# thierrydumas/autoencoder_based_image_compression

Measured on AMD Instinct MI355X. Metric: Mpixels/s encode+decode (Kodak 768x512 luma), bitstream bit-exact, higher is better.
Workload: dtype f32; 1 GPU; kodak_512x768_luma_batch24_per_gpu_bin_width_1.0_lossless_roundtrip; height=512, width=768, truncated_unary_length=10, idx_map_exception=67, parallelism=single GPU, coder=device, 64 maps per wavefront, encode + decode + compare

## Files before the change

autoencoder_based_image_compression_amd/csrc/hip/coder_simd.hip:

```cpp
#include <hip/hip_runtime.h>
#include <stdint.h>

#include <mutex>

#include "../coder/lean_step.h"
#include "eae_hip.h"
#include "fill.h"
#include "wave_scan.h"

int eae_coder_generic_encode(uint32_t n_maps, uint32_t map_size, const int16_t* symbols, uint8_t L, const double* probs,
                             const int32_t* prob_row, uint8_t* streams, uint64_t stride, uint32_t* bac_bits,
                             uint32_t* bypass_bits, int32_t* status, int32_t* stage, int only_status, hipStream_t stream);
int eae_coder_generic_decode(uint32_t n_maps, uint32_t map_size, int16_t* out, uint8_t L, const double* probs,
                             const int32_t* prob_row, const uint8_t* streams, uint64_t stride, const uint32_t* bac_bits,
                             const uint32_t* bypass_bits, int32_t* status, int32_t* stage, int only_status, hipStream_t stream);

#ifndef EAE_RES_BINARISE
#define EAE_RES_BINARISE 47
#endif
#ifndef EAE_RES_ENCODE_CORE
#define EAE_RES_ENCODE_CORE 55
#endif
#ifndef EAE_RES_EMIT
#define EAE_RES_EMIT 39
#endif
#ifndef EAE_RES_DECODE_CORE
#define EAE_RES_DECODE_CORE 55
#endif
#ifndef EAE_RES_DEBINARISE
#define EAE_RES_DEBINARISE 23
#endif
#ifndef EAE_RES_DEBINARISE_STAGED
#define EAE_RES_DEBINARISE_STAGED 39
#endif
#ifndef EAE_RES_DECODE_CORE_CHUNKED
#define EAE_RES_DECODE_CORE_CHUNKED 63
#endif
#ifndef EAE_DECODE_TOPUP_ZEROS
#define EAE_KEEP_VGPR_FREE_(n) asm volatile("; v" #n " reserved: the last register of the allocation holds no operand" ::: "v" #n)
#define EAE_KEEP_LAST_VGPR_FREE(n) EAE_KEEP_VGPR_FREE_(n)
#else
#define EAE_KEEP_LAST_VGPR_FREE(n)
#endif

namespace {

using namespace eae_core;
using namespace eae_lean;


#ifndef EAE_SIMD_PRIO
#define EAE_SIMD_PRIO 3
#endif

constexpr int32_t RETRY = -100;
constexpr uint32_t kMaxFastL = 32;
constexpr uint32_t kRecordPad = 12;
constexpr uint32_t kRing = 32;
constexpr uint32_t kBypassStage = 512;
constexpr uint32_t kDebinariseStage = 1024;
constexpr uint32_t kEmitWords = 224;

struct SimdParams {
    uint32_t n_maps, map_size, L, dcap;
    uint32_t rcap;
    const int16_t* symbols;
    int16_t* decoded;
    const double* probs;
    const int32_t* prob_row;
    uint8_t* streams;
    uint64_t stride;
    uint32_t* bac_bits;
    uint32_t* bypass_bits;
    int32_t* status;
    int32_t* stage;
    uint8_t* decisions;
    uint32_t* ndec;
    uint32_t* records;
    uint8_t* prefixes;
    uint32_t chunk, nchunks;
    uint32_t* group_steps;
    uint2* enc_state;
    uint4* emit_state;
    uint32_t* avail_bits;
    uint4* dec_state;
    uint2* dec_state2;
};

__host__ __device__ inline uint32_t chunk_span(uint32_t steps, uint32_t nchunks) {
    const uint32_t span = ((steps + nchunks - 1u) / nchunks + 63u) & ~63u;
    return span ? span : 64u;
}

__device__ __forceinline__ int wave_exclusive_max(int v) {
    int m = __builtin_amdgcn_update_dpp(-1, v, 0x138, 0xF, 0xF, false);
#define EAE_MAX_STEP(ctrl_, rows_)                                                        \
    {                                                                                     \
        const int o_ = __builtin_amdgcn_update_dpp(-1, m, ctrl_, rows_, 0xF, false);      \
        m = o_ > m ? o_ : m;                                                              \
    }
    EAE_MAX_STEP(0x111, 0xF)
    EAE_MAX_STEP(0x112, 0xF)
    EAE_MAX_STEP(0x114, 0xF)
    EAE_MAX_STEP(0x118, 0xF)
    EAE_MAX_STEP(0x142, 0xA)
    EAE_MAX_STEP(0x143, 0xC)
#undef EAE_MAX_STEP
    return m;
}
__device__ __forceinline__ uint32_t wave_max(uint32_t v) {
#pragma unroll
    for (int d = 32; d >= 1; d >>= 1) {
        const uint32_t o = __shfl_xor(v, d, 64);
        v = o > v ? o : v;
    }
    return v;
}

__global__ __launch_bounds__(64) void binarise_kernel(const SimdParams p) {
    EAE_KEEP_LAST_VGPR_FREE(EAE_RES_BINARISE);
    __shared__ unsigned long long ybuf[40];
    const uint32_t m = blockIdx.x, lane = threadIdx.x;
    const int32_t row = p.prob_row ? p.prob_row[m] : (int32_t)m;
    if (row < 0) {
        if (lane == 0) { p.ndec[m] = 0; p.bac_bits[m] = 0; p.bypass_bits[m] = 0; p.status[m] = 0; if (p.stage) p.stage[m] = 0; }
        return;
    }
    const uint32_t L = p.L;
    const int16_t* in = p.symbols + (size_t)m * p.map_size;
    uint8_t* dec = p.decisions + (size_t)(m >> 6) * 64u * p.dcap + (size_t)(m & 63u) * 8u;
    unsigned long long* ystream = reinterpret_cast<unsigned long long*>(p.streams + (uint64_t)m * p.stride + p.stride / 2);
    const uint32_t size_bits = round_up_to_byte(required_bits(p.map_size, L));
    uint32_t jbase = 0, bbase = 0;
    bool overflow = false;
    if (lane < 40) ybuf[lane] = 0;
    for (uint32_t t = 0; t < p.map_size; t += 64) {
        const uint32_t i = t + lane;
        const bool valid = i < p.map_size;
        const int s = valid ? (int)in[i] : 0;
        const uint32_t a = (uint32_t)(s < 0 ? -s : s);
        const uint32_t ones = a < L ? a : L;
        const uint32_t nd = valid ? ones + (a < L ? 1u : 0u) : 0u;
        unsigned long long bb = 0;
        uint32_t nb = 0;
        if (valid && a >= L) {
            const uint32_t v = a - L + 1u;
            const uint32_t n = count_nb_bits(v) - 1u;
            bb = ((1ull << n) - 1ull) | ((unsigned long long)(n ? rev16(v - (1u << n)) >> (16u - n) : 0u) << (n + 1u));
            nb = 2u * n + 1u;
        }
        if (valid && s != 0) {
            bb |= (unsigned long long)(s > 0 ? 1u : 0u) << nb;
            nb++;
        }
        uint32_t both_tot;
        const uint32_t both = wave_exclusive_scan(nd | (nb << 16), both_tot);
        const uint32_t jo = both & 0xFFFFu, bo = both >> 16, jtot = both_tot & 0xFFFFu, btot = both_tot >> 16;
        for (uint32_t q = 0; q < nd; q++) {
            const uint32_t j = jbase + jo + q;
            dec[(size_t)(j >> 3) * 512u + (j & 7u)] = (uint8_t)((q << 1) | (q < ones ? 1u : 0u));
        }
        if (nb) {
            const uint32_t pos = (bbase & 63u) + bo;
            atomicOr(&ybuf[pos >> 6], bb << (pos & 63u));
            if ((pos & 63u) + nb > 64u) atomicOr(&ybuf[(pos >> 6) + 1u], bb >> (64u - (pos & 63u)));
        }
        if (bbase + btot > size_bits) overflow = true;
        if (overflow) break;
        const uint32_t nfull = ((bbase & 63u) + btot) >> 6;
        const unsigned long long mine = lane < 40 ? ybuf[lane] : 0ull;
        const unsigned long long carry = ybuf[nfull];
        if (lane < nfull) ystream[(bbase >> 6) + lane] = mine;
        if (lane < 40) ybuf[lane] = lane == 0 ? carry : 0ull;
        jbase += jtot;
        bbase += btot;
    }
    if (lane == 0) {
        if (!overflow && (bbase & 63u)) ystream[bbase >> 6] = ybuf[0];
        p.ndec[m] = jbase;
        p.bypass_bits[m] = bbase;
        p.bac_bits[m] = 0;
        p.status[m] = overflow ? RETRY : 0;
        if (p.stage) p.stage[m] = 0;
    }
}

extern __shared__ double lds_dyn[];

template <bool CHUNKED>
__global__ __launch_bounds__(64) void bac_encode_core_kernel(const SimdParams p) {
    EAE_KEEP_LAST_VGPR_FREE(EAE_RES_ENCODE_CORE);
    __builtin_amdgcn_s_setprio(EAE_SIMD_PRIO);
    const uint32_t lane = threadIdx.x;
    const uint32_t m = blockIdx.x * 64u + lane;
    const bool in_range = m < p.n_maps;
    const int32_t row = in_range ? (p.prob_row ? p.prob_row[m] : (int32_t)m) : -1;
    const bool live = in_range && row >= 0 && p.status[m] == 0;
    const uint32_t L = p.L;
    double* probs = lds_dyn;
    bool retry = false;
    if (live)
        for (uint32_t k = 0; k < L; k++) {
            const double pk = p.probs[(size_t)row * L + k];
            probs[k * 64u + lane] = scale_probability(pk);
            if (!(pk > 0. && pk < 1.)) retry = true;
        }
    const uint32_t nd = live && !retry ? p.ndec[m] : 0u;
    uint32_t steps = wave_max(nd);
    const uint32_t nd_all = ~wave_max(~(nd ? nd : 0xFFFFFFFFu));
    const uint8_t* dec = p.decisions + (size_t)blockIdx.x * 64u * p.dcap + (size_t)lane * 8u;
    uint32_t* rec = p.records + (size_t)(in_range ? m : 0u) * p.rcap;
    Interval s = interval_init();
    uint32_t j_first = 0;
    if (CHUNKED) {
        if (p.chunk == 0u) { if (lane == 0u) p.group_steps[blockIdx.x] = steps; }
        else steps = p.group_steps[blockIdx.x];
        const uint32_t span = chunk_span(steps, p.nchunks);
        j_first = p.chunk * span < steps ? p.chunk * span : steps;
        steps = j_first + span < steps ? j_first + span : steps;
        if (p.chunk != 0u && in_range) { const uint2 st = p.enc_state[m]; s.lo = st.x; s.hc = st.y; }
    }
    const uint32_t last_round = (steps ? steps - 1u : 0u) >> 3;
    auto decisions_of = [&](uint32_t round) __attribute__((always_inline)) {
        return *reinterpret_cast<const uint2*>(dec + (size_t)(round < last_round ? round : last_round) * 512u);
    };
    uint32_t* const sink = rec + p.dcap + 8u;
    const uint32_t nd_here = CHUNKED ? (nd < steps ? nd : steps) : nd;
    auto round_of_eight = [&](const uint2& d, uint32_t jb) __attribute__((always_inline)) {
        const unsigned long long d8 = (unsigned long long)d.x | ((unsigned long long)d.y << 32);
        auto probability = [&](uint32_t q) __attribute__((always_inline)) {
            const uint32_t ctx = (uint32_t)(d8 >> (8u * q + 1u)) & 31u;
            return probs[(ctx < L ? ctx : 0u) * 64u + lane];
        };
        uint32_t r[8];
        if (jb + 8u <= nd_all && jb + 8u <= steps) {
            double pq[8];
#pragma unroll
            for (uint32_t q = 0; q < 8; q++) pq[q] = probability(q);
#pragma unroll
            for (uint32_t q = 0; q < 8; q++) r[q] = encode_step(s, pq[q], ((uint32_t)(d8 >> (8u * q)) & 1u) != 0u);
        } else {
#pragma unroll
            for (uint32_t q = 0; q < 8; q++) {
                const Interval before = s;
                const uint32_t rec_q = encode_step(s, probability(q), ((uint32_t)(d8 >> (8u * q)) & 1u) != 0u);
                const bool has = jb + q < nd_here;
                s.lo = has ? s.lo : before.lo;
                s.hc = has ? s.hc : before.hc;
                r[q] = has ? rec_q : 0u;
            }
        }
        *reinterpret_cast<uint4*>(jb < nd_here ? rec + jb : sink) = make_uint4(r[0], r[1], r[2], r[3]);
        *reinterpret_cast<uint4*>(jb + 4u < nd_here ? rec + jb + 4u : sink) = make_uint4(r[4], r[5], r[6], r[7]);
    };
    uint2 da = decisions_of(j_first >> 3), db = decisions_of((j_first >> 3) + 1u), dc = decisions_of((j_first >> 3) + 2u);
    __builtin_amdgcn_s_waitcnt(0x0F70);
    for (uint32_t jb = j_first; jb < steps; jb += 24) {
        const uint32_t round = jb >> 3;
        round_of_eight(da, jb);
        da = decisions_of(round + 3u);
        round_of_eight(db, jb + 8u);
        db = decisions_of(round + 4u);
        round_of_eight(dc, jb + 16u);
        dc = decisions_of(round + 5u);
    }
    if (live) {
        if (retry) p.status[m] = RETRY;
        else if (!CHUNKED || p.chunk + 1u == p.nchunks) rec[nd] = stop_record(s);
        else p.enc_state[m] = make_uint2(s.lo, s.hc);
    }
}

template <bool CHUNKED>
__global__ __launch_bounds__(64) void emit_kernel(const SimdParams p) {
    EAE_KEEP_LAST_VGPR_FREE(EAE_RES_EMIT);
    __shared__ unsigned long long buf[kEmitWords + 2];
    const uint32_t m = blockIdx.x, lane = threadIdx.x;
    const int32_t row = p.prob_row ? p.prob_row[m] : (int32_t)m;
    if (row < 0 || p.status[m] != 0) return;
    uint32_t nrec = p.ndec[m] + 1u;
    const uint32_t* rec = p.records + (size_t)m * p.rcap;
    unsigned long long* out = reinterpret_cast<unsigned long long*>(p.streams + (uint64_t)m * p.stride);
    const uint32_t size_bits = round_up_to_byte(required_bits(p.map_size, p.L));
    for (uint32_t w = lane; w < kEmitWords + 2u; w += 64u) buf[w] = 0ull;
    uint32_t base = 0, pending = 0;
    bool give_up = false;
    uint32_t t_first = 0;
    const bool last_chunk = !CHUNKED || p.chunk + 1u == p.nchunks;
    if (CHUNKED) {
        const uint32_t span = chunk_span(p.group_steps[m >> 6], p.nchunks);
        const uint32_t nd = nrec - 1u;
        t_first = p.chunk * span < nd ? p.chunk * span : nd;
        if (!last_chunk) nrec = t_first + span < nd ? t_first + span : nd;
        if (p.chunk != 0u) {
            const uint4 st = p.emit_state[m];
            base = st.x;
            pending = st.y;
            if (lane == 0) buf[0] = (unsigned long long)st.z | ((unsigned long long)st.w << 32);
        }
    }
    for (uint32_t t = t_first; t < nrec; t += 4u * 64u) {
        const uint32_t j0 = t + 4u * lane;
        uint4 rr = make_uint4(0u, 0u, 0u, 0u);
        if (j0 < nrec) rr = *reinterpret_cast<const uint4*>(rec + j0);
        uint32_t r[4] = {rr.x, rr.y, rr.z, rr.w};
        uint32_t n[4], k[4], kl[4];
        bool has[4];
        uint32_t ksum = 0;
#pragma unroll
        for (uint32_t q = 0; q < 4; q++) {
            if (j0 + q >= nrec) r[q] = 0u;
            n[q] = record_n(r[q]);
            k[q] = record_k(r[q]);
            has[q] = n[q] != 0u;
            kl[q] = ksum;
            ksum += k[q];
        }
        uint32_t ktot;
        const uint32_t e0 = wave_exclusive_scan(ksum, ktot);
        int lane_last = -1;
#pragma unroll
        for (uint32_t q = 0; q < 4; q++) lane_last = has[q] ? (int)(e0 + kl[q]) : lane_last;
        const int below = wave_exclusive_max(lane_last);
        uint32_t c[4], cl[4], queue[4];
        uint32_t csum = 0;
        int since = below;
#pragma unroll
        for (uint32_t q = 0; q < 4; q++) {
            const uint32_t e = e0 + kl[q];
            queue[q] = (since >= 0 ? e - (uint32_t)since : pending + e) + (record_is_stop(r[q]) ? 1u : 0u);
            c[q] = has[q] ? n[q] + queue[q] : 0u;
            cl[q] = csum;
            csum += c[q];
            since = has[q] ? (int)e : since;
        }
        uint32_t ctot;
        const uint32_t o0 = wave_exclusive_scan(csum, ctot);
        const int tile_last = __builtin_amdgcn_readlane(since, 63);
        pending = tile_last >= 0 ? ktot - (uint32_t)tile_last : pending + ktot;
        const uint32_t start = base & 63u;
        if (start + ctot > kEmitWords * 64u || base + ctot > size_bits) { give_up = true; break; }
#pragma unroll
        for (uint32_t q = 0; q < 4; q++) {
            if (has[q]) {
                const uint32_t lead = record_leaving(r[q]);
                const unsigned long long first = lead >> 31;
                const unsigned long long rest = (unsigned long long)(__builtin_bitreverse32(lead << 1) & ((1u << (n[q] - 1u)) - 1u));
                const uint32_t pos = start + o0 + cl[q];
                const uint32_t qu = queue[q];
                if (c[q] <= 64u) {
                    const unsigned long long run = first ? 0ull : (((qu < 63u ? (1ull << qu) : (1ull << 63)) - 1ull) | (qu == 63u ? (1ull << 62) : 0ull));
                    const unsigned long long v = first | (run << 1) | (qu + 1u < 64u ? rest << (qu + 1u) : 0ull);
                    const uint32_t sh = pos & 63u;
                    atomicOr(&buf[pos >> 6], v << sh);
                    if (sh + c[q] > 64u) atomicOr(&buf[(pos >> 6) + 1u], v >> (64u - sh));
                } else {
                    if (first) atomicOr(&buf[pos >> 6], 1ull << (pos & 63u));
                    if (!first) {
                        uint32_t b0 = pos + 1u;
                        const uint32_t b1 = pos + 1u + qu;
                        while (b0 < b1) {
                            const uint32_t sh = b0 & 63u;
                            const uint32_t cnt = (b1 - b0) < (64u - sh) ? (b1 - b0) : (64u - sh);
                            const unsigned long long ones = cnt == 64u ? ~0ull : (((1ull << cnt) - 1ull) << sh);
                            atomicOr(&buf[b0 >> 6], ones);
                            b0 += cnt;
                        }
                    }
                    const uint32_t pr = pos + 1u + qu, sh = pr & 63u;
                    if (rest) {
                        atomicOr(&buf[pr >> 6], rest << sh);
                        if (sh + (n[q] - 1u) > 64u) atomicOr(&buf[(pr >> 6) + 1u], rest >> (64u - sh));
                    }
                }
            }
        }
        const uint32_t nfull = (start + ctot) >> 6;
        for (uint32_t w = lane; w < nfull; w += 64u) out[(base >> 6) + w] = buf[w];
        const unsigned long long carry = buf[nfull];
        for (uint32_t w = lane; w <= nfull; w += 64u) buf[w] = 0ull;
        if (lane == 0) buf[0] = carry;
        base += ctot;
    }
    if (lane == 0) {
        if (give_up) {
            p.status[m] = RETRY;
        } else if (last_chunk) {
            if (base & 63u) out[base >> 6] = buf[0];
            p.bac_bits[m] = base;
        } else {
            const unsigned long long carry = buf[0];
            p.emit_state[m] = make_uint4(base, pending, (uint32_t)carry, (uint32_t)(carry >> 32));
            p.avail_bits[m] = base & ~63u;
        }
    }
}

constexpr size_t decode_lds_bytes(uint32_t L) { return ((size_t)L + 1u) * 64u * sizeof(double) + ((size_t)kRing + 1u) * 64u * sizeof(uint32_t); }

#ifdef EAE_HWID_PROBE
__device__ unsigned int g_hwid_probe[8];
#endif

constexpr uint32_t kNotStarted = 0xFFFFFFFFu;
constexpr uint32_t kStepMargin = 46u;

template <bool CHUNKED>
__global__ __launch_bounds__(64) void bac_decode_core_kernel(const SimdParams p) {
    if (CHUNKED) { EAE_KEEP_LAST_VGPR_FREE(EAE_RES_DECODE_CORE_CHUNKED); } else { EAE_KEEP_LAST_VGPR_FREE(EAE_RES_DECODE_CORE); }
    __builtin_amdgcn_s_setprio(EAE_SIMD_PRIO);
#ifdef EAE_HWID_PROBE
    const unsigned int probe_hw0 = __builtin_amdgcn_s_getreg(((32 - 1) << 11) | (0 << 6) | 4);
    const unsigned int probe_xcc0 = __builtin_amdgcn_s_getreg(((4 - 1) << 11) | (0 << 6) | 20);
#endif
    const uint32_t lane = threadIdx.x;
    const uint32_t m = blockIdx.x * 64u + lane;
    const bool in_range = m < p.n_maps;
    const int32_t row = in_range ? (p.prob_row ? p.prob_row[m] : (int32_t)m) : -1;
    const uint32_t L = p.L;
    double* probs = lds_dyn;
    uint32_t* ring = reinterpret_cast<uint32_t*>(lds_dyn + ((size_t)L + 1u) * 64u) + lane;
    const bool live = in_range && row >= 0 && p.status[m] == 0;
    const bool final_chunk = !CHUNKED || p.chunk + 1u == p.nchunks;
    const uint32_t nbac = live ? (final_chunk ? p.bac_bits[m] : p.avail_bits[m]) : 0u;
    bool retry = false;
    if (live && (nbac > p.stride * 4u || p.bypass_bits[m] > p.stride * 4u)) retry = true;
    if (live) {
        for (uint32_t k = 0; k < L; k++) {
            const double pk = p.probs[(size_t)row * L + k];
            probs[k * 64u + lane] = scale_probability(pk);
            if (!(pk > 0. && pk < 1.)) retry = true;
        }
        probs[L * 64u + lane] = scale_probability(0.5);
    }
    const uint32_t size = live && !retry ? p.map_size : 0u;
    const uint4* src = reinterpret_cast<const uint4*>(p.streams + (uint64_t)(in_range ? m : 0u) * p.stride);
    const uint32_t nwords = size ? (nbac + 31u) >> 5 : 0u;
    uint4 parked = make_uint4(0u, 0u, 0u, kNotStarted);
    uint2 parked2 = make_uint2(0u, 0u);
    if (CHUNKED && size) { parked = p.dec_state[m]; parked2 = p.dec_state2[m]; }
    const bool started = CHUNKED && parked.w != kNotStarted;
    const uint32_t taken0 = started ? parked.w : 0u;
    const uint32_t word0 = taken0 >> 5, wbase = word0 & ~3u;
#ifdef EAE_DECODE_TOPUP_ZEROS
    auto fetch = [&](uint32_t w0) {
        uint4 v = make_uint4(0u, 0u, 0u, 0u);
        if (w0 < nwords) v = src[w0 >> 2];
        v.x = w0 + 0u < nwords ? __builtin_bitreverse32(v.x) : 0u;
        v.y = w0 + 1u < nwords ? __builtin_bitreverse32(v.y) : 0u;
        v.z = w0 + 2u < nwords ? __builtin_bitreverse32(v.z) : 0u;
        v.w = w0 + 3u < nwords ? __builtin_bitreverse32(v.w) : 0u;
        return v;
    };
    auto land = [&](uint32_t w0, const uint4& v) {
        ring[((w0 + 0u) & (kRing - 1u)) * 64u] = v.x;
        ring[((w0 + 1u) & (kRing - 1u)) * 64u] = v.y;
        ring[((w0 + 2u) & (kRing - 1u)) * 64u] = v.z;
        ring[((w0 + 3u) & (kRing - 1u)) * 64u] = v.w;
    };
#pragma unroll
    for (uint32_t w0 = 0; w0 < kRing; w0 += 4u) land(w0, fetch(w0));
#else
    auto fetch = [&](uint32_t w0) {
        uint4 v = make_uint4(0u, 0u, 0u, 0u);
        if (w0 < nwords) v = src[w0 >> 2];
        return v;
    };
    auto land = [&](uint32_t w0, const uint4& v) {
        ring[((w0 + 0u) & (kRing - 1u)) * 64u] = __builtin_bitreverse32(v.x);
        ring[((w0 + 1u) & (kRing - 1u)) * 64u] = __builtin_bitreverse32(v.y);
        ring[((w0 + 2u) & (kRing - 1u)) * 64u] = __builtin_bitreverse32(v.z);
        ring[((w0 + 3u) & (kRing - 1u)) * 64u] = __builtin_bitreverse32(v.w);
        if ((w0 & (kRing - 1u)) == 0u) ring[kRing * 64u] = __builtin_bitreverse32(v.x);
    };
    {
        uint4 first[kRing / 4u];
#pragma unroll
        for (uint32_t g = 0; g < kRing / 4u; g++) first[g] = fetch(wbase + 4u * g);
#pragma unroll
        for (uint32_t g = 0; g < kRing / 4u; g++) land(wbase + 4u * g, first[g]);
    }
#endif
    uint32_t loaded = wbase + kRing;
    unsigned long long rwin = (((unsigned long long)ring[(word0 & (kRing - 1u)) * 64u] << 32) |
                               (unsigned long long)ring[((word0 + 1u) & (kRing - 1u)) * 64u]) << (taken0 & 31u);
    uint32_t rcount = 64u - (taken0 & 31u), rword = word0 + 2u;
    uint32_t left = nbac > taken0 ? nbac - taken0 : 0u;
    uint32_t code32 = parked.z;
    bool begun = started;
    if (!started && (final_chunk || left >= kStepMargin)) {
        const uint32_t k = left < 16u ? left : 16u;
        uint32_t bits = (uint32_t)((rwin >> 1) >> (63u - k));
        const uint32_t sticky = bits & 1u;
        bits = (bits << (16u - k)) | (sticky ? ((1u << (16u - k)) - 1u) : 0u);
        rwin <<= k;
        rcount -= k;
        left -= k;
        code32 = bits << 16;
        begun = true;
    }
    Interval s = interval_init();
    const double p0 = probs[lane];
    double pk = p0;
    uint32_t unary = 0, i = 0;
    if (started) {
        s.lo = parked.x;
        s.hc = parked.y;
        unary = parked2.x;
        i = parked2.y;
        pk = probs[unary * 64u + lane];
    }
    uint8_t* prefix = p.prefixes + (size_t)(in_range ? m : 0u) * p.map_size;
    const uint32_t steps_left_any = wave_max(size);
    uint4 fa = make_uint4(0u, 0u, 0u, 0u), fb = fa;
    bool flying = false;
    if (steps_left_any) {
        for (;;) {
            if (flying) {
                land(loaded, fa);
                land(loaded + 4u, fb);
                loaded += 8u;
            }
#ifdef EAE_DECODE_TOPUP_ZEROS
            flying = loaded - rword <= kRing - 8u;
#else
            flying = loaded - rword <= kRing - 10u && loaded < nwords;
#endif
            if (flying) {
                fa = fetch(loaded);
                fb = fetch(loaded + 4u);
            }
#ifdef EAE_DECODE_TOPUP_ZEROS
            bool fast_round = false;
#else
            bool fast_round = !__any(size != 0u && i + 8u > size) && (!CHUNKED || final_chunk || !__any(size != 0u && !begun));
#endif
            if (fast_round) {
                if (size) {
                    const uint32_t bp0 = rword * 32u - rcount;
                    uint32_t bp = bp0;
                    const Interval s0 = s;
                    const uint32_t code0 = code32, unary0 = unary, i0 = i;
                    const double pk0 = pk;
#pragma unroll
                    for (uint32_t q = 0; q < 8; q++) {
                        const uint32_t row = (bp >> 5) & (kRing - 1u);
                        const uint32_t hi = ring[row * 64u], lo = ring[row * 64u + 64u];
                        const double pspec = probs[(unary + 1u) * 64u + lane];
                        const DecodeStep d = decode_step(s, code32, pk);
                        const uint32_t win = (uint32_t)(((((unsigned long long)hi << 32) | (unsigned long long)lo) << (bp & 31u)) >> 32);
                        const uint32_t bits = (win >> 1) >> (31u - d.take);
                        bp += d.take;
                        code32 = shift_code(code32, d, bits);
                        const uint32_t count = unary + (d.one ? 1u : 0u);
                        prefix[i] = (uint8_t)count;
                        const bool done = !d.one || count == L;
                        i += done ? 1u : 0u;
                        unary = done ? 0u : count;
                        pk = done ? p0 : pspec;
                    }
                    if (__any(bp - bp0 > left)) {
                        s = s0; code32 = code0; unary = unary0; i = i0; pk = pk0;
                        fast_round = false;
                    } else {
                        left -= bp - bp0;
                        const uint32_t row = (bp >> 5) & (kRing - 1u);
                        rwin = (((unsigned long long)ring[row * 64u] << 32) | (unsigned long long)ring[row * 64u + 64u]) << (bp & 31u);
                        rcount = 64u - (bp & 31u);
                        rword = (bp >> 5) + 2u;
                    }
                }
            }
            if (!fast_round) {
#pragma unroll
            for (uint32_t q = 0; q < 8; q++) {
                if (i < size && (!CHUNKED || final_chunk || (begun && left >= kStepMargin))) {
                    const uint32_t wnext = ring[(rword & (kRing - 1u)) * 64u];
                    const double pspec = probs[(unary + 1u) * 64u + lane];
                    const bool need = rcount <= 32u;
                    rwin |= (unsigned long long)(need ? wnext : 0u) << (need ? 32u - rcount : 0u);
                    rcount += need ? 32u : 0u;
                    rword += need ? 1u : 0u;
                    const DecodeStep d = decode_step(s, code32, pk);
                    const uint32_t k = d.take < left ? d.take : left;
                    uint32_t bits = (uint32_t)((rwin >> 1) >> (63u - k));
                    const uint32_t ext = d.take - k;
                    bits = (bits << ext) | ((bits & 1u) ? ((1u << ext) - 1u) : 0u);
                    rwin <<= k;
                    rcount -= k;
                    left -= k;
                    code32 = shift_code(code32, d, bits);
                    const bool done = !d.one || unary + 1u == L;
                    if (done) prefix[i] = (uint8_t)(d.one ? L : unary);
                    i += done ? 1u : 0u;
                    unary = done ? 0u : unary + 1u;
                    pk = done ? p0 : pspec;
                }
            }
            }
            if (!__any(i < size && (!CHUNKED || final_chunk || (begun && left >= kStepMargin)))) break;
        }
    }
    if (CHUNKED && size && !final_chunk) {
        p.dec_state[m] = make_uint4(s.lo, s.hc, code32, begun ? nbac - left : kNotStarted);
        p.dec_state2[m] = make_uint2(unary, i);
    }
    if (live && retry) p.status[m] = RETRY;
#ifdef EAE_HWID_PROBE
    {
        const unsigned int hw1 = __builtin_amdgcn_s_getreg(((32 - 1) << 11) | (0 << 6) | 4);
        const unsigned int xcc1 = __builtin_amdgcn_s_getreg(((4 - 1) << 11) | (0 << 6) | 20);
        if (lane == 0) {
            atomicAdd(&g_hwid_probe[0], 1u);
            if (((hw1 ^ probe_hw0) & 0xFFFFu) != 0u || xcc1 != probe_xcc0) {
                atomicAdd(&g_hwid_probe[1], 1u);
                g_hwid_probe[2] = probe_hw0; g_hwid_probe[3] = probe_xcc0; g_hwid_probe[4] = hw1; g_hwid_probe[5] = xcc1;
            }
        }
    }
#endif
}

#ifdef EAE_HWID_PROBE
extern "C" int eae_hip_debug_hwid_probe(unsigned int* out8) {
    return (int)hipMemcpyFromSymbol(out8, HIP_SYMBOL(g_hwid_probe), 8 * sizeof(unsigned int));
}
#endif

template <bool STAGED>
__global__ __launch_bounds__(64) void debinarise_kernel(const SimdParams p) {
    if (STAGED) { EAE_KEEP_LAST_VGPR_FREE(EAE_RES_DEBINARISE_STAGED); } else { EAE_KEEP_LAST_VGPR_FREE(EAE_RES_DEBINARISE); }
    __shared__ uint32_t ytile[80];
    const uint32_t m = blockIdx.x, lane = threadIdx.x;
    const int32_t row = p.prob_row ? p.prob_row[m] : (int32_t)m;
    if (lane == 0 && p.ndec) p.ndec[m] = 0u;
    if (row < 0 || p.status[m] != 0) {
        if (row >= 0 && p.status[m] == RETRY && lane == 0 && p.ndec) p.ndec[m] = 1u;
        return;
    }
    const uint32_t L = p.L, size = p.map_size;
    const uint32_t nbyp = p.bypass_bits[m];
    const uint32_t* gbyp = reinterpret_cast<const uint32_t*>(p.streams + (uint64_t)m * p.stride + p.stride / 2);
    const uint32_t ywords = (nbyp + 31u) >> 5;
    const uint8_t* prefix = p.prefixes + (size_t)m * size;
    const int16_t* expected = p.symbols ? p.symbols + (size_t)m * size : nullptr;
    int16_t* out = p.decoded ? p.decoded + (size_t)m * size : nullptr;
    uint32_t ybase = 0;
    bool bad = false, differ = false;
    __shared__ uint32_t ystage[STAGED ? kBypassStage + 80u : 1u];
    __shared__ uint8_t pstage[STAGED ? kDebinariseStage : 1u];
    __shared__ int16_t estage[STAGED ? kDebinariseStage : 1u];
    if (STAGED) {
        const uint32_t have = ywords < kBypassStage ? ywords : kBypassStage, last = ywords ? ywords - 1u : 0u;
        for (uint32_t k = 0; k < have; k += 512u) {
            uint32_t v[8];
#pragma unroll
            for (uint32_t u = 0; u < 8; u++) {
                const uint32_t w = k + u * 64u + lane;
                v[u] = gbyp[w < last ? w : last];
            }
#pragma unroll
            for (uint32_t u = 0; u < 8; u++) {
                const uint32_t w = k + u * 64u + lane;
                if (w < kBypassStage) ystage[w] = w < ywords ? v[u] : 0u;
            }
        }
        for (uint32_t w = have + lane; w < kBypassStage + 80u; w += 64u) ystage[w] = 0u;
    }
    for (uint32_t t = 0; t < size; t += 64u) {
        if (STAGED && (t & (kDebinariseStage - 1u)) == 0u) {
            const uint32_t last = size - 1u;
            __syncthreads();
            for (uint32_t k = 0; k < kDebinariseStage && t + k < size; k += 512u) {
                uint8_t pv[8];
                int16_t ev[8];
#pragma unroll
                for (uint32_t u = 0; u < 8; u++) {
                    const uint32_t i = t + k + u * 64u + lane, at_i = i < last ? i : last;
                    pv[u] = prefix[at_i];
                    ev[u] = expected ? expected[at_i] : (int16_t)0;
                }
#pragma unroll
                for (uint32_t u = 0; u < 8; u++) {
                    pstage[k + u * 64u + lane] = pv[u];
                    estage[k + u * 64u + lane] = ev[u];
                }
            }
            __syncthreads();
        }
        const uint32_t w0 = ybase >> 5;
        const bool in_stage = STAGED && (ywords <= kBypassStage ? w0 <= kBypassStage : w0 + 80u <= kBypassStage);
        if (!in_stage) {
            ytile[lane] = w0 + lane < ywords ? gbyp[w0 + lane] : 0u;
            if (lane < 16u) ytile[64u + lane] = w0 + 64u + lane < ywords ? gbyp[w0 + 64u + lane] : 0u;
        }
        const uint32_t* const window = in_stage ? ystage + w0 : ytile;
        auto bits_at = [&](uint32_t pos) {
            const uint32_t rel = pos - (w0 << 5), q = rel >> 5, sh = rel & 31u;
            const unsigned long long two = (unsigned long long)window[q] | ((unsigned long long)window[q + 1u] << 32);
            return (uint32_t)(two >> sh);
        };
        const uint32_t i = t + lane;
        const bool valid = i < size;
        uint32_t a = valid ? (uint32_t)(STAGED ? pstage[i & (kDebinariseStage - 1u)] : prefix[i]) : 0u;
        const bool nonzero = a != 0u;
        uint32_t ntot;
        uint32_t at = wave_exclusive_scan(nonzero ? 1u : 0u, ntot);
        uint32_t extra = 0;
        unsigned long long escapes = __ballot(valid && a == L);
        uint32_t extra_tot = 0;
        while (escapes) {
            const int e = __builtin_ctzll(escapes);
            escapes &= escapes - 1ull;
            const uint32_t pos = ybase + (uint32_t)__builtin_amdgcn_readlane((int)at, e) + extra_tot;
            const uint32_t w = bits_at(pos);
            const uint32_t nn = (uint32_t)__builtin_ctz(~w | 0x80000000u);
            if (nn > 16u || pos + 2u * nn + 1u > nbyp) { bad = true; break; }
            const uint32_t suffix = nn ? __builtin_bitreverse32(bits_at(pos + nn + 1u)) >> (32u - nn) : 0u;
            const uint32_t value = (L + ((suffix + (1u << nn) - 1u) & 0xFFFFu)) & 0xFFFFu;
            const uint32_t len = 2u * nn + 1u;
            if ((int)lane == e) a = value;
            if ((int)lane >= e) extra += len;
            extra_tot += len;
        }
        if (bad) break;
        const uint32_t spos = ybase + at + extra;
        if (nonzero && spos >= nbyp) bad = true;
        if (__any(bad)) { bad = true; break; }
        int v = (int)(int16_t)a;
        if (nonzero && !(bits_at(spos) & 1u)) v = -v;
        if (valid) {
            if (out) out[i] = (int16_t)v;
            if (expected && (STAGED ? estage[i & (kDebinariseStage - 1u)] : expected[i]) != (int16_t)v) differ = true;
        }
        ybase += ntot + extra_tot;
    }
    const bool any_differ = __any(differ);
    if (lane == 0) {
        if (bad) { p.status[m] = RETRY; if (p.ndec) p.ndec[m] = 1u; }
        else if (expected && any_differ) p.status[m] = MISMATCH;
    }
}

__global__ __launch_bounds__(64) void compare_kernel(const SimdParams p) {
    const uint32_t m = blockIdx.x, lane = threadIdx.x;
    if (p.ndec[m] == 0u) return;
    const int32_t row = p.prob_row ? p.prob_row[m] : (int32_t)m;
    if (row < 0 || p.status[m] != 0) return;
    const int16_t* a = p.symbols + (size_t)m * p.map_size;
    const int16_t* b = p.decoded + (size_t)m * p.map_size;
    int differ = 0;
    for (uint32_t i = lane; i < p.map_size; i += 64) differ |= (a[i] != b[i]);
    if (__any(differ) && lane == 0) p.status[m] = MISMATCH;
}

#ifdef EAE_EXPERIMENTAL_CODER
constexpr uint32_t kPipeRecords = 64u;
constexpr uint32_t kPipeSpinLimit = 1u << 21;
constexpr uint32_t kPipeDone = 0x80000000u, kPipeBad = 0x40000000u;

#define EAE_PIPE_ORDER() asm volatile("s_waitcnt lgkmcnt(0)" ::: "memory")

constexpr size_t pipe_lds_bytes(uint32_t L) {
    return ((size_t)L + 1u) * 64u * sizeof(double) + ((size_t)kPipeRecords + kRing) * 64u * sizeof(uint32_t) + (8u + 4u * 64u) * sizeof(uint32_t);
}

#ifndef EAE_RES_PIPE
#define EAE_RES_PIPE 63
#endif

#ifdef EAE_PIPE_PROBE
__device__ unsigned long long g_pipe_probe[3][4];
__device__ unsigned long long g_pipe_probe2[8];
#define PIPE_T0() const long long probe_t0 = clock64(); long long probe_wait = 0, probe_mark = 0; unsigned probe_rounds = 0
#define PIPE_WAIT_BEGIN() probe_mark = clock64()
#define PIPE_WAIT_END() probe_wait += clock64() - probe_mark
#define PIPE_ROUND() probe_rounds++
#define PIPE_REPORT(role_) if (blockIdx.x == 0 && lane == 0) { g_pipe_probe[role_][0] = clock64() - probe_t0; g_pipe_probe[role_][1] = probe_wait; \
    g_pipe_probe[role_][2] = probe_rounds; g_pipe_probe[role_][3] = __builtin_amdgcn_s_getreg(((32 - 1) << 11) | (0 << 6) | 4); }
#else
#define PIPE_T0()
#define PIPE_WAIT_BEGIN()
#define PIPE_WAIT_END()
#define PIPE_ROUND()
#define PIPE_REPORT(role_)
#endif

__global__ __launch_bounds__(256) void coder_pipe_kernel(const SimdParams p) {
    EAE_KEEP_LAST_VGPR_FREE(EAE_RES_PIPE);
    const uint32_t tid = threadIdx.x, lane = tid & 63u;
    const uint32_t role = (uint32_t)__builtin_amdgcn_readfirstlane((int)(tid >> 6));
    const uint32_t m = blockIdx.x * 64u + lane;
    const bool in_range = m < p.n_maps;
    const int32_t row = in_range ? (p.prob_row ? p.prob_row[m] : (int32_t)m) : -1;
    const uint32_t L = p.L;
    double* probs = lds_dyn;
    uint32_t* recring = reinterpret_cast<uint32_t*>(lds_dyn + ((size_t)L + 1u) * 64u);
    uint32_t* wring = recring + kPipeRecords * 64u;
    volatile uint32_t* ctl = wring + kRing * 64u;
    volatile uint32_t* lane_ok = ctl + 8;
    volatile uint32_t* wr_words = lane_ok + 64;
    volatile uint32_t* wr_bits = wr_words + 64;
    volatile uint32_t* rd_word = wr_bits + 64;
    const bool live = in_range && row >= 0 && p.status[m] == 0;
    __builtin_amdgcn_s_setprio(EAE_SIMD_PRIO);
    if (role == 0u) {
        bool good = live;
        if (live) {
            for (uint32_t k = 0; k < L; k++) {
                const double pk = p.probs[(size_t)row * L + k];
                probs[k * 64u + lane] = scale_probability(pk);
                if (!(pk > 0. && pk < 1.)) good = false;
            }
            probs[L * 64u + lane] = scale_probability(0.5);
        }
        lane_ok[lane] = good ? 1u : 0u;
        wr_words[lane] = 0u;
        wr_bits[lane] = 0u;
        rd_word[lane] = 0u;
        if (lane < 8u) ctl[lane] = 0u;
    }
    __syncthreads();
    if (role == 3u) return;
    const bool good = lane_ok[lane] != 0u;
    const uint32_t nd = good ? p.ndec[m] : 0u;

    PIPE_T0();
    if (role == 0u) {
        const uint32_t steps = wave_max(nd);
        const uint32_t nd_all = ~wave_max(~(nd ? nd : 0xFFFFFFFFu));
        const uint8_t* dec = p.decisions + (size_t)blockIdx.x * 64u * p.dcap + (size_t)lane * 8u;
        Interval s = interval_init();
        uint2 ahead = steps ? *reinterpret_cast<const uint2*>(dec) : make_uint2(0, 0);
        bool gave_up = false;
        auto wait_for_room = [&](uint32_t upto) {
            uint32_t spins = 0;
            for (;;) {
                EAE_PIPE_ORDER();
                const uint32_t slowest = ctl[2];
                if (slowest == 0xFFFFFFFFu || upto <= slowest + kPipeRecords) return true;
                if (ctl[3] != 0u || ++spins > kPipeSpinLimit) return false;
                __builtin_amdgcn_s_sleep(2);
            }
        };
        for (uint32_t jb = 0; jb < steps; jb += 8) {
            PIPE_WAIT_BEGIN();
            const bool room_ok = wait_for_room(jb + 8u);
            PIPE_WAIT_END();
            PIPE_ROUND();
            if (!room_ok) { gave_up = true; break; }
            const unsigned long long d8 = (unsigned long long)ahead.x | ((unsigned long long)ahead.y << 32);
            if (jb + 8 < steps) ahead = *reinterpret_cast<const uint2*>(dec + (size_t)((jb >> 3) + 1u) * 512u);
            double pq[8];
#pragma unroll
            for (uint32_t q = 0; q < 8; q++) {
                const uint32_t ctx = (uint32_t)(d8 >> (8u * q + 1u)) & 31u;
                pq[q] = probs[(ctx < L ? ctx : 0u) * 64u + lane];
            }
            uint32_t r[8];
            if (jb + 8u <= nd_all) {
#pragma unroll
                for (uint32_t q = 0; q < 8; q++) r[q] = encode_step(s, pq[q], ((uint32_t)(d8 >> (8u * q)) & 1u) != 0u);
            } else {
#pragma unroll
                for (uint32_t q = 0; q < 8; q++) {
                    r[q] = 0u;
                    if (jb + q < nd) r[q] = encode_step(s, pq[q], ((uint32_t)(d8 >> (8u * q)) & 1u) != 0u);
                }
            }
#pragma unroll
            for (uint32_t q = 0; q < 8; q++)
                if (jb + q < nd) recring[((jb + q) & (kPipeRecords - 1u)) * 64u + lane] = r[q];
            EAE_PIPE_ORDER();
            if (lane == 0u) ctl[0] = jb + 8u;
        }
        if (!gave_up && !wait_for_room(steps + 1u)) gave_up = true;
        if (!gave_up) {
            if (nd) recring[(nd & (kPipeRecords - 1u)) * 64u + lane] = stop_record(s);
            EAE_PIPE_ORDER();
            if (lane == 0u) ctl[1] = 1u;
        } else if (lane == 0u) {
            ctl[3] = 1u;
        }
        if (live && !good) p.status[m] = RETRY;
        PIPE_REPORT(0);
        return;
    }

    if (role == 1u) {
        uint32_t* out = reinterpret_cast<uint32_t*>(p.streams + (uint64_t)(in_range ? m : 0u) * p.stride);
        const uint32_t size_bits = round_up_to_byte(required_bits(p.map_size, L));
        uint32_t j = 0, cnt = 0, nwords = 0, pending = 0, total = 0;
        unsigned long long acc = 0ull;
        bool fin = nd == 0u, bad = false;
        uint32_t spins = 0;
        bool gave_up = false;
        auto flush = [&]() {
            const uint32_t word = (uint32_t)acc;
            wring[(nwords & (kRing - 1u)) * 64u + lane] = __builtin_bitreverse32(word);
            out[nwords] = word;
            acc >>= 32;
            cnt -= 32u;
            nwords++;
        };
        for (;;) {
            EAE_PIPE_ORDER();
            const uint32_t have = ctl[0], stopped = ctl[1], taken_words = rd_word[lane];
            const uint32_t ordinary = j < nd ? (have < nd ? have : nd) - j : 0u;
            const uint32_t ready = ordinary + ((j + ordinary == nd && stopped != 0u) ? 1u : 0u);
            const uint32_t slots = taken_words + kRing - nwords;
            uint32_t limit = ready < 8u ? ready : 8u;
            limit = limit + 3u <= slots ? limit : (slots > 3u ? slots - 3u : 0u);
            if (fin || bad) limit = 0u;
            const bool progressed = limit != 0u;
#pragma unroll
            for (uint32_t q = 0; q < 8; q++) {
                const uint32_t gom = q < limit ? 0xFFFFFFFFu : 0u;
                const uint32_t r = recring[(j & (kPipeRecords - 1u)) * 64u + lane];
                const uint32_t n = record_n(r), k = record_k(r), stop = (r >> 4) & 1u;
                const uint32_t queue = pending + stop;
                const uint32_t hasm = n != 0u ? gom : 0u;
                const uint32_t first = r >> 31;
                const uint32_t rest = __builtin_amdgcn_ubfe(__builtin_bitreverse32(r << 1), 0u, n - 1u);
                const uint32_t odd = (queue > 15u || total + n + queue > size_bits) ? hasm : 0u;
                if (__any(odd != 0u)) {
                    if (odd != 0u && (total + n + queue > size_bits || queue > 64u)) bad = true;
                    if (hasm != 0u && !bad) {
                        acc |= (unsigned long long)first << cnt;
                        cnt += 1u;
                        if (cnt >= 32u) flush();
                        for (uint32_t left_run = queue; left_run != 0u;) {
                            const uint32_t t = left_run < 16u ? left_run : 16u;
                            acc |= (unsigned long long)(first ? 0u : ((1u << t) - 1u)) << cnt;
                            cnt += t;
                            if (cnt >= 32u) flush();
                            left_run -= t;
                        }
                        acc |= (unsigned long long)rest << cnt;
                        cnt += n - 1u;
                        if (cnt >= 32u) flush();
                        total += n + queue;
                        if (queue > 15u) limit = q + 1u;
                    }
                } else {
                    const uint32_t run = (first - 1u) & ((1u << (queue & 31u)) - 1u);
                    const uint32_t v = (first | (run << 1) | (rest << ((queue + 1u) & 31u))) & hasm;
                    const uint32_t c = (n + queue) & hasm;
                    acc |= (unsigned long long)v << cnt;
                    cnt += c;
                    total += c;
                    if (cnt >= 32u) flush();
                }
                pending = gom != 0u ? (n != 0u ? k : pending + k) : pending;
                j -= gom;
                if (__any((gom & stop) != 0u)) {
                    if ((gom & stop) != 0u && !bad) {
                        if (cnt) { cnt = 32u; flush(); }
                        fin = true;
                        p.bac_bits[m] = total;
                    }
                }
            }
            wr_bits[lane] = total;
            EAE_PIPE_ORDER();
            wr_words[lane] = nwords | (fin ? kPipeDone : 0u) | (bad ? kPipeBad : 0u);
            const uint32_t mine = (!fin && !bad && j < nd) ? j : 0xFFFFFFFFu;
            const uint32_t slowest = ~wave_max(~mine);
            if (lane == 0u) ctl[2] = slowest;
            if (!__any(!fin && !bad)) break;
            PIPE_ROUND();
            if (__any(progressed)) spins = 0;
            else {
                if (ctl[3] != 0u || ++spins > kPipeSpinLimit) { gave_up = true; break; }
                PIPE_WAIT_BEGIN();
                __builtin_amdgcn_s_sleep(2);
                PIPE_WAIT_END();
            }
        }
        PIPE_REPORT(1);
        if (gave_up && lane == 0u) ctl[3] = 1u;
        if (good && (bad || gave_up || ctl[3] != 0u)) p.status[m] = RETRY;
        return;
    }

    uint32_t* ring = wring + lane;
    const uint32_t size = good ? p.map_size : 0u;
    Interval s = interval_init();
    const double p0 = probs[lane];
    double pk = p0;
    uint32_t unary = 0, i = 0, taken = 0, code32 = 0, rcount = 0, rword = 0;
    unsigned long long rwin = 0ull;
    bool begun = false, dropped = size == 0u;
#ifdef EAE_PIPE_PROBE
    bool probe_seen_complete = false;
    unsigned probe_fast = 0, probe_lost = 0, probe_waits = 0;
#endif
    uint8_t* prefix = p.prefixes + (size_t)(in_range ? m : 0u) * p.map_size;
    uint32_t spins = 0;
    for (;;) {
        EAE_PIPE_ORDER();
        const uint32_t w = wr_words[lane];
        const bool complete = (w & kPipeDone) != 0u;
        if (w & kPipeBad) dropped = true;
        EAE_PIPE_ORDER();
        const uint32_t avail = complete ? wr_bits[lane] : (w & 0x3FFFFFFFu) * 32u;
        bool progressed = false;
#ifdef EAE_PIPE_PROBE
        if (blockIdx.x == 0 && !probe_seen_complete && !__any(!dropped && !complete)) {
            probe_seen_complete = true;
            if (lane == 0) { g_pipe_probe2[0] = probe_rounds; g_pipe_probe2[1] = clock64() - probe_t0; }
        }
#endif
        const bool fed = complete || avail - taken >= kStepMargin + 64u;
        const bool crowded = !dropped && i < size && avail - taken >= 16u * 32u;
        if (__any(!dropped && i < size && !fed) && !__any(crowded)) {
            if (ctl[3] != 0u || ++spins > kPipeSpinLimit) { if (lane == 0u) ctl[3] = 1u; break; }
            PIPE_WAIT_BEGIN();
            __builtin_amdgcn_s_sleep(4);
            PIPE_WAIT_END();
            continue;
        }
        spins = 0;
        if (!dropped && !begun && (complete || avail >= 64u)) {
            rwin = ((unsigned long long)ring[0] << 32) | (unsigned long long)ring[64];
            rcount = 64u;
            rword = 2u;
            const uint32_t k = avail < 16u ? avail : 16u;
            uint32_t bits = (uint32_t)((rwin >> 1) >> (63u - k));
            const uint32_t sticky = bits & 1u;
            bits = (bits << (16u - k)) | (sticky ? ((1u << (16u - k)) - 1u) : 0u);
            rwin <<= k;
            rcount -= k;
            taken = k;
// ... 382 lines not shown
```

Before: 3020 Mpixels/s.

## Pack decisions in LDS, add escape-free fast paths for binarise, emit and debinarise

The binarise kernel now builds decision bytes in a shared 64-bit row buffer with packed odd-valued patterns and writes whole 8-byte rows, replacing per-byte scattered global stores. It also takes a ballot/mbcnt fast path when no lane in the wave hits the escape code, so only sign bits are placed. The BAC emit loop merges a lane's four records into one 64-bit word when their total fits, and debinarise uses ballot counts plus direct global sign reads when a tile has no escapes. These changes add branches and LDS atomics, and they rely on the packed decision layout exactly matching what the byte writes produced before.

```diff
diff --git a/autoencoder_based_image_compression_amd/csrc/hip/coder_simd.hip b/autoencoder_based_image_compression_amd/csrc/hip/coder_simd.hip
--- a/autoencoder_based_image_compression_amd/csrc/hip/coder_simd.hip
+++ b/autoencoder_based_image_compression_amd/csrc/hip/coder_simd.hip
@@ -117,9 +117,16 @@
     return v;
 }
 
+__device__ __forceinline__ uint32_t wave_count_below(unsigned long long mask) {
+    return __builtin_amdgcn_mbcnt_hi((uint32_t)(mask >> 32), __builtin_amdgcn_mbcnt_lo((uint32_t)mask, 0u));
+}
+
+constexpr uint32_t kDecisionRows = (7u + 64u * kMaxFastL + 7u) / 8u;
+
 __global__ __launch_bounds__(64) void binarise_kernel(const SimdParams p) {
     EAE_KEEP_LAST_VGPR_FREE(EAE_RES_BINARISE);
     __shared__ unsigned long long ybuf[40];
+    __shared__ unsigned long long dbuf[kDecisionRows + 1u];
     const uint32_t m = blockIdx.x, lane = threadIdx.x;
     const int32_t row = p.prob_row ? p.prob_row[m] : (int32_t)m;
     if (row < 0) {
@@ -128,12 +135,13 @@
     }
     const uint32_t L = p.L;
     const int16_t* in = p.symbols + (size_t)m * p.map_size;
-    uint8_t* dec = p.decisions + (size_t)(m >> 6) * 64u * p.dcap + (size_t)(m & 63u) * 8u;
+    unsigned long long* drow = reinterpret_cast<unsigned long long*>(p.decisions + (size_t)(m >> 6) * 64u * p.dcap + (size_t)(m & 63u) * 8u);
     unsigned long long* ystream = reinterpret_cast<unsigned long long*>(p.streams + (uint64_t)m * p.stride + p.stride / 2);
     const uint32_t size_bits = round_up_to_byte(required_bits(p.map_size, L));
     uint32_t jbase = 0, bbase = 0;
     bool overflow = false;
     if (lane < 40) ybuf[lane] = 0;
+    for (uint32_t w = lane; w < kDecisionRows + 1u; w += 64u) dbuf[w] = 0ull;
     for (uint32_t t = 0; t < p.map_size; t += 64) {
         const uint32_t i = t + lane;
         const bool valid = i < p.map_size;
@@ -141,32 +149,66 @@
         const uint32_t a = (uint32_t)(s < 0 ? -s : s);
         const uint32_t ones = a < L ? a : L;
         const uint32_t nd = valid ? ones + (a < L ? 1u : 0u) : 0u;
-        unsigned long long bb = 0;
-        uint32_t nb = 0;
-        if (valid && a >= L) {
-            const uint32_t v = a - L + 1u;
-            const uint32_t n = count_nb_bits(v) - 1u;
-            bb = ((1ull << n) - 1ull) | ((unsigned long long)(n ? rev16(v - (1u << n)) >> (16u - n) : 0u) << (n + 1u));
-            nb = 2u * n + 1u;
-        }
-        if (valid && s != 0) {
-            bb |= (unsigned long long)(s > 0 ? 1u : 0u) << nb;
-            nb++;
-        }
-        uint32_t both_tot;
-        const uint32_t both = wave_exclusive_scan(nd | (nb << 16), both_tot);
-        const uint32_t jo = both & 0xFFFFu, bo = both >> 16, jtot = both_tot & 0xFFFFu, btot = both_tot >> 16;
-        for (uint32_t q = 0; q < nd; q++) {
-            const uint32_t j = jbase + jo + q;
-            dec[(size_t)(j >> 3) * 512u + (j & 7u)] = (uint8_t)((q << 1) | (q < ones ? 1u : 0u));
-        }
-        if (nb) {
-            const uint32_t pos = (bbase & 63u) + bo;
-            atomicOr(&ybuf[pos >> 6], bb << (pos & 63u));
-            if ((pos & 63u) + nb > 64u) atomicOr(&ybuf[(pos >> 6) + 1u], bb >> (64u - (pos & 63u)));
-        }
-        if (bbase + btot > size_bits) overflow = true;
-        if (overflow) break;
+        uint32_t jo, jtot, btot;
+        if (__ballot(a >= L) == 0ull) {
+            const unsigned long long nonzero = __ballot(s != 0);
+            jo = wave_exclusive_scan(nd, jtot);
+            btot = (uint32_t)__builtin_popcountll(nonzero);
+            if (s > 0) {
+                const uint32_t pos = (bbase & 63u) + wave_count_below(nonzero);
+                atomicOr(&ybuf[pos >> 6], 1ull << (pos & 63u));
+            }
+        } else {
+            unsigned long long bb = 0;
+            uint32_t nb = 0;
+            if (valid && a >= L) {
+                const uint32_t v = a - L + 1u;
+                const uint32_t n = count_nb_bits(v) - 1u;
+                bb = ((1ull << n) - 1ull) | ((unsigned long long)(n ? rev16(v - (1u << n)) >> (16u - n) : 0u) << (n + 1u));
+                nb = 2u * n + 1u;
+            }
+            if (s != 0) {
+                bb |= (unsigned long long)(s > 0 ? 1u : 0u) << nb;
+                nb++;
+            }
+            uint32_t both_tot;
+            const uint32_t both = wave_exclusive_scan(nd | (nb << 16), both_tot);
+            jo = both & 0xFFFFu;
+            jtot = both_tot & 0xFFFFu;
+            btot = both_tot >> 16;
+            if (nb) {
+                const uint32_t pos = (bbase & 63u) + (both >> 16);
+                atomicOr(&ybuf[pos >> 6], bb << (pos & 63u));
+                if ((pos & 63u) + nb > 64u) atomicOr(&ybuf[(pos >> 6) + 1u], bb >> (64u - (pos & 63u)));
+            }
+        }
+        if (bbase + btot > size_bits) { overflow = true; break; }
+        if (a != 0u) {
+            const uint32_t pos = (jbase & 7u) + jo;
+            const uint32_t sh = (pos & 7u) * 8u;
+            uint32_t w = pos >> 3;
+            unsigned long long odd = 0x0F0D0B0907050301ull;
+            for (uint32_t k = 0; k < nd; k += 8u) {
+                const uint32_t cnt = ones - k;
+                unsigned long long v = odd;
+                if (cnt < 8u) {
+                    v &= (1ull << (8u * cnt)) - 1ull;
+                    if (a < L) v |= (unsigned long long)(2u * a) << (8u * cnt);
+                }
+                atomicOr(&dbuf[w], v << sh);
+                if (sh) atomicOr(&dbuf[w + 1u], v >> (64u - sh));
+                odd += 0x1010101010101010ull;
+                w++;
+            }
+        }
+        {
+            const uint32_t nrows = ((jbase & 7u) + jtot) >> 3;
+            unsigned long long* const dst = drow + (size_t)(jbase >> 3) * 64u;
+            for (uint32_t w = lane; w < nrows; w += 64u) dst[(size_t)w * 64u] = dbuf[w];
+            const unsigned long long carry = dbuf[nrows];
+            for (uint32_t w = lane; w <= nrows; w += 64u) dbuf[w] = 0ull;
+            if (lane == 0) dbuf[0] = carry;
+        }
         const uint32_t nfull = ((bbase & 63u) + btot) >> 6;
         const unsigned long long mine = lane < 40 ? ybuf[lane] : 0ull;
         const unsigned long long carry = ybuf[nfull];
@@ -176,6 +218,7 @@
         bbase += btot;
     }
     if (lane == 0) {
+        if (jbase & 7u) drow[(size_t)(jbase >> 3) * 64u] = dbuf[0];
         if (!overflow && (bbase & 63u)) ystream[bbase >> 6] = ybuf[0];
         p.ndec[m] = jbase;
         p.bypass_bits[m] = bbase;
@@ -340,6 +383,26 @@
         pending = tile_last >= 0 ? ktot - (uint32_t)tile_last : pending + ktot;
         const uint32_t start = base & 63u;
         if (start + ctot > kEmitWords * 64u || base + ctot > size_bits) { give_up = true; break; }
+        if (csum <= 64u) {
+            if (csum) {
+                unsigned long long joined = 0ull;
+#pragma unroll
+                for (uint32_t q = 0; q < 4; q++) {
+                    if (has[q]) {
+                        const uint32_t lead = record_leaving(r[q]);
+                        const unsigned long long first = lead >> 31;
+                        const unsigned long long rest = (unsigned long long)(__builtin_bitreverse32(lead << 1) & ((1u << (n[q] - 1u)) - 1u));
+                        const uint32_t qu = queue[q];
+                        const unsigned long long run = first ? 0ull : (((qu < 63u ? (1ull << qu) : (1ull << 63)) - 1ull) | (qu == 63u ? (1ull << 62) : 0ull));
+                        const unsigned long long v = first | (run << 1) | (qu + 1u < 64u ? rest << (qu + 1u) : 0ull);
+                        joined |= v << cl[q];
+                    }
+                }
+                const uint32_t pos = start + o0, sh = pos & 63u;
+                atomicOr(&buf[pos >> 6], joined << sh);
+                if (sh + csum > 64u) atomicOr(&buf[(pos >> 6) + 1u], joined >> (64u - sh));
+            }
+        } else {
 #pragma unroll
         for (uint32_t q = 0; q < 4; q++) {
             if (has[q]) {
@@ -375,6 +438,7 @@
                 }
             }
         }
+        }
         const uint32_t nfull = (start + ctot) >> 6;
         for (uint32_t w = lane; w < nfull; w += 64u) out[(base >> 6) + w] = buf[w];
         const unsigned long long carry = buf[nfull];
@@ -688,9 +752,17 @@
             }
             __syncthreads();
         }
+        const uint32_t i = t + lane;
+        const bool valid = i < size;
+        uint32_t a = valid ? (uint32_t)(STAGED ? pstage[i & (kDebinariseStage - 1u)] : prefix[i]) : 0u;
+        const bool nonzero = a != 0u;
+        const unsigned long long signs = __ballot(nonzero);
+        const uint32_t at = wave_count_below(signs), ntot = (uint32_t)__builtin_popcountll(signs);
+        unsigned long long escapes = __ballot(valid && a == L);
         const uint32_t w0 = ybase >> 5;
         const bool in_stage = STAGED && (ywords <= kBypassStage ? w0 <= kBypassStage : w0 + 80u <= kBypassStage);
-        if (!in_stage) {
+        const bool direct = !STAGED && escapes == 0ull;
+        if (!in_stage && !direct) {
             ytile[lane] = w0 + lane < ywords ? gbyp[w0 + lane] : 0u;
             if (lane < 16u) ytile[64u + lane] = w0 + 64u + lane < ywords ? gbyp[w0 + 64u + lane] : 0u;
         }
@@ -700,14 +772,7 @@
             const unsigned long long two = (unsigned long long)window[q] | ((unsigned long long)window[q + 1u] << 32);
             return (uint32_t)(two >> sh);
         };
-        const uint32_t i = t + lane;
-        const bool valid = i < size;
-        uint32_t a = valid ? (uint32_t)(STAGED ? pstage[i & (kDebinariseStage - 1u)] : prefix[i]) : 0u;
-        const bool nonzero = a != 0u;
-        uint32_t ntot;
-        uint32_t at = wave_exclusive_scan(nonzero ? 1u : 0u, ntot);
         uint32_t extra = 0;
-        unsigned long long escapes = __ballot(valid && a == L);
         uint32_t extra_tot = 0;
         while (escapes) {
             const int e = __builtin_ctzll(escapes);
@@ -728,7 +793,10 @@
         if (nonzero && spos >= nbyp) bad = true;
         if (__any(bad)) { bad = true; break; }
         int v = (int)(int16_t)a;
-        if (nonzero && !(bits_at(spos) & 1u)) v = -v;
+        uint32_t sign;
+        if (direct) sign = nonzero ? gbyp[spos >> 5] >> (spos & 31u) : 1u;
+        else sign = bits_at(spos);
+        if (nonzero && !(sign & 1u)) v = -v;
         if (valid) {
             if (out) out[i] = (int16_t)v;
             if (expected && (STAGED ? estage[i & (kDebinariseStage - 1u)] : expected[i]) != (int16_t)v) differ = true;
```

After: 3002 Mpixels/s. About the same (-0.6%).
